# plus-rkwitt/flooder

Measured on AMD Instinct MI355X. Metric: M points×simplices/s (coverage sweep), higher is better.
Workload: dtype f32; 1 GPU; 1M-point 3D Gaussian, 1k landmarks, points_per_edge 30, max_dimension 3, fp32 coverage sweep (BASELINE.json configs[1]); points=1000000, landmarks=1000, top_simplices=6052, top_simplices_rank0=6052, swept_dimension=3, method=cell, parallelism=single GPU

## Files before the change

### flooder_amd/_native.py

```python

from __future__ import annotations

import ctypes
import os
from ctypes import c_char_p, c_float, c_int, c_int32, c_int64, c_uint32, c_void_p

_PKG_DIR = os.path.dirname(os.path.abspath(__file__))
LIB_PATH = os.environ.get("FLOODER_HIP_LIB") or os.path.join(_PKG_DIR, "libflooder_hip.so")



class _Block(ctypes.Structure):

    ABI = 1

    def __init__(self, **fields):
        super().__init__()
        self.size = ctypes.sizeof(self)
        self.abi = self.ABI
        known = {name for name, _ in self._fields_}
        for key, value in fields.items():
            if key not in known:
                raise TypeError(f"{type(self).__name__} has no field {key!r}")
            if value is not None and not isinstance(value, (int, float)):
# ... 8 lines not shown
        item = item.strip()
        if item:
            kind, name = item.split()
            out.append((name, kinds[kind]))
    return out


class FusedSweep(_Block):

    _fields_ = _fields("""u32 size; u32 abi; p pts_sorted; i64 n_pts; i32 dim; i32 k1; p nodes; p density_grid; p cloud_box;
        p verts; p weights; i32 R; i32 n_faces; i64 n_simplices; p memb; f32 alpha; i32 n_coarse; p coarse_rows; p parents;
        p face_bits; p face_slot; p d2_scratch; p flag_list; p flag_count; p flag_key; p flag_hist; p flag_sorted; p top;
        p top_list; p top_count; p simplex_weight; p plane_scratch; p wit_queue; p wit_item_list; p wit_stats;
        p cell_queue; p defer_list; p defer_c; p defer_ctl; p light_list; p heavy_list; p cell_stats; p finish_ctl;
        p hard_scratch; i32 hard_cap; i32 probed; p finish_stats; p wit_runs; i32 wit_run_len; i32 wit_n_runs;
        i32 planes_ready; i32 reserved; p face_owner; p min_face; p chunk_faces; p tile_faces""")


class SortedSweep(_Block):

    _fields_ = _fields("""u32 size; u32 abi; p pts_sorted; i64 n_pts; i32 dim; i32 k1; p nodes; p verts; p weights; i32 R;
        i32 n_faces; i64 n_simplices; p sample_order; p queue; p memb; p face_bits; p face_slot; p stats; p out_d2;
        i32 shard_rank; i32 shard_world""")


class FpsBatched(_Block):

    _fields_ = _fields("""u32 size; u32 abi; p pts; i64 n_pts; i32 dim; i32 ld; p pts_sorted; p order; i64 start; i32 n_lms;
        i32 reserved; p out_idx; p minsq; p bucket_box; p bucket_keys; p bucket_coord; p work_best; p work_rec; p work_ctr;
        p launches_out""")

# ... 291 lines not shown
```

### flooder_amd/core.py

```python

from __future__ import annotations

import ctypes
import itertools
import math
import os
import weakref
import warnings
from numbers import Integral, Real
from typing import Callable, Dict, List, NamedTuple, Optional, Tuple, Union

import numpy as np
import torch

from . import _native
from .simplex_tree import HAS_GUDHI, SimplexTree, delaunay_cells, delaunay_simplices

__all__ = ["flood_complex", "generate_landmarks", "generate_grid", "generate_uniform_weights",
           "SUPPORTED_DTYPES", "HAS_HIP_KERNELS", "PointIndex", "index_from_host"]

SUPPORTED_DTYPES = (torch.float32, torch.float64)
INF_BITS = 0x7F800000
CAND_ALIGN = 8
SWEEP_CHUNK = 2048
# ... 859 lines not shown
    par = (nn[:, 0] | (nn[:, 1] << 8) | (nn[:, 2] << 16) | (nn[:, 3] << 24)).astype(np.uint32)
    rows = np.full(WIT_MAX_COARSE, -1, dtype=np.int32)
    rows[:coarse.size] = inv[coarse]
    out = (rows, np.ascontiguousarray(par[np.asarray(perm)]), int(coarse.size))
    if len(_WIT_PLAN_CACHE) >= 32:
        _WIT_PLAN_CACHE.clear()
    _WIT_PLAN_CACHE[key] = out
    return out


WIT_RUN_LEN = 8
WIT_RUN_SUM_TOL = 2.0 ** -21


def witness_runs(w_perm: np.ndarray, memb: np.ndarray, parents: np.ndarray,
                 run_len: Optional[int] = None) -> Optional[np.ndarray]:
    run_len = WIT_RUN_LEN if run_len is None else int(run_len)
    w32 = np.ascontiguousarray(w_perm, dtype=np.float32)
    R, k1 = w32.shape
    n = R // run_len
    if k1 > 4 or n == 0 or run_len < 8 or run_len & (run_len - 1) or (w32 < 0).any():
        return None
    w = w32.astype(np.float64)[:n * run_len].reshape(n, run_len, k1)
    c = w.mean(axis=1)
    rows = np.arange(n)
    for it in range(1, 65):
        far = ((w - c[:, None, :]) ** 2).sum(axis=2).argmax(axis=1)
        c += (w[rows, far] - c) / (it + 1)
    c32 = np.maximum(c, 0.0).astype(np.float32)
    c64 = c32.astype(np.float64)
    d = np.sqrt(((w - c64[:, None, :]) ** 2).sum(axis=2))
    rho = d.max(axis=1) * (1.0 + 1e-12)
    rho32 = rho.astype(np.float32)
    rho32 = np.where(rho32.astype(np.float64) < rho, np.nextafter(rho32, np.float32(np.inf)), rho32).astype(np.float32)
    sums = w32.astype(np.float64).sum(axis=1)
    if max(np.abs(sums - 1.0).max(), np.abs(c64.sum(axis=1) - 1.0).max()) > 0.5 * WIT_RUN_SUM_TOL:
        return None
    out = np.zeros((n, 8), dtype=np.uint32)
    out[:, :k1] = c32.view(np.uint32)
    out[:, 4] = np.bitwise_or.reduce(np.asarray(memb).view(np.uint32)[:n * run_len].reshape(n, run_len), axis=1)
    out[:, 5] = np.asarray(parents).view(np.uint32)[:n * run_len].reshape(n, run_len)[rows, d.argmin(axis=1)]
    out[:, 6] = rho32.view(np.uint32)
    return out


def face_lattice(weights: np.ndarray, f_ptr: np.ndarray, f_rows: np.ndarray) -> Optional[Tuple[np.ndarray, np.ndarray]]:
    w = np.asarray(weights)
    R, k1 = w.shape
    F = len(f_ptr) - 1
    if F > 32 or k1 > 31:
        return None
    supp = ((w != 0) * (1 << np.arange(k1))).sum(axis=1).astype(np.int64)
    vset = np.array([np.bitwise_or.reduce(supp[f_rows[f_ptr[f]:f_ptr[f + 1]]]) if f_ptr[f + 1] > f_ptr[f] else 0
                     for f in range(F)], dtype=np.int64)
    if len(set(vset.tolist())) != F or (vset == 0).any():
        return None
    holds = (supp[:, None] & ~vset[None, :]) == 0
# ... 78 lines not shown
        if not self._wit_built:
            self._wit_built = True
            wp = witness_plan(self._weights, self._perm) if self.memb_all is not None else None
            if wp is not None:
                dev = self._weights.device
                self._wit = (torch.as_tensor(wp[0], device=dev), torch.as_tensor(wp[1].view(np.int32), device=dev), wp[2])
        return self._wit


    @property
    def wit_runs(self):
        if not self._wit_runs_built:
            self._wit_runs_built = True
            if self.wit is not None:
                run_len = WIT_RUN_LEN
                tab = witness_runs(self.w_perm.cpu().numpy(), self.memb_all.cpu().numpy(), self.wit[1].cpu().numpy(), run_len)
                if tab is not None:
                    self._wit_runs = (torch.as_tensor(tab.view(np.int32), device=self._weights.device), run_len,
                                      int(tab.shape[0]))
        return self._wit_runs


def _sweep_dimension_f64(index: PointIndex, pts64_sorted: torch.Tensor, verts: torch.Tensor, weights: torch.Tensor,
                         faces: _FaceTable, reduce_hook: Optional[Callable[[torch.Tensor], None]],
                         want_dist: bool = False, timer: Optional[_KernelTimer] = None):
    lib = _native.load()
    dev = index.pts.device
    st = _native.current_stream_ptr(dev)
    S, k1, _ = verts.shape
    R = weights.shape[0]
    verts = verts.to(torch.float64).contiguous()
# ... 488 lines not shown
BVH_SORTED_MIN_SAMPLES = 64 * 1024
EMPTY_CACHE_ABOVE_BYTES = 1 << 30
CELL_ALPHA = 1.35
FUSED_FACES = True
CELL_PROBE = True
SHARED_FACE_SLOTS = True
FINISH_HARD_CAP = 32768
CELL_DENSITY_GRID = True
CELL_SUPER = True
WIT_MIN_SIMPLICES = 1536
WIT_MAX_POINTS_PER_SIMPLEX = 400
CELL_WITNESS = True
WIT_RUNS = True
FACE_OWNER = True
FACE_OWNER_GROUPED = False

CTL_FLAG_COUNT, CTL_DEFER, CTL_HIST = 1, 12, 48


def fused_layout(S: int, n_slots: int, wit: bool, owner: bool) -> Tuple[Dict[str, Tuple[int, int]], int]:
    sizes = [("wit_queue", QUEUE_WORDS)] if wit else []
    sizes += [("cell_queue", _native.CELL_QUEUE_WORDS), ("finish_ctl", _native.FINISH_CTL_WORDS), ("top", 2 * S),
              ("ctl", CTL_HIST + _native.FLAG_HIST_WORDS), ("face_bits", n_slots)]
    if owner:
        sizes += [("face_owner", 2 * n_slots), ("result", n_slots)]
    regions, n_words = {}, 0
    for name, words in sizes:
        if name == "face_owner":
            n_words += n_words & 1
        regions[name] = (n_words, words)
# ... 79 lines not shown
                                                              k1, S, _native.ptr(ws.wgt), _native.ptr(ws.planes),
                                                              _native.ptr(ws.arena), ws.n_words, st),
                              "flooder_simplex_prepare_f32")
            else:
                _native.check(lib.flooder_simplex_weight_f32(_native.ptr(index.nodes), index.n, index.dim, _native.ptr(verts),
                                                             k1, S, _native.ptr(ws.wgt), st), "flooder_simplex_weight_f32")
        wst = stats[16:40] if use_wit and stats is not None and stats.numel() >= 40 else None
        blk = _native.FusedSweep(
            pts_sorted=index.pts, n_pts=index.n, dim=index.dim, k1=k1, nodes=index.nodes, density_grid=index.dens,
            cloud_box=index.box, verts=verts, weights=w_perm, R=R, n_faces=F, n_simplices=S, memb=plan.memb_all,
            alpha=float(CELL_ALPHA), face_slot=slot_t, cell_stats=sub(0, 9), probed=1 if CELL_PROBE else 0,
            finish_stats=sub(9, 16), **ws.block_fields())
        if use_owner:
            blk.min_face = plan.min_face.data_ptr()
            blk.chunk_faces, blk.tile_faces = plan.chunk_faces.data_ptr(), plan.tile_faces.data_ptr()
        if use_wit:
            blk.n_coarse, blk.coarse_rows, blk.parents = plan.wit[2], plan.wit[0].data_ptr(), plan.wit[1].data_ptr()
            blk.wit_stats = _native.ptr(wst) or None
            if WIT_RUNS and plan.wit_runs is not None:
                blk.wit_runs, blk.wit_run_len, blk.wit_n_runs = plan.wit_runs[0].data_ptr(), plan.wit_runs[1], plan.wit_runs[2]
        blk.planes_ready = 1 if CELL_SUPER and SWEEP_PREPARE_FUSED else 0
        with _span(timer, "sweep"):
            if use_wit:
                _native.check(lib.flooder_fused_witness(ctypes.byref(blk), st), "flooder_fused_witness")
                blk.planes_ready = 1
            _native.check(lib.flooder_fused_cell(ctypes.byref(blk), st), "flooder_fused_cell")
        with _span(timer, "fallback"):
            _native.check(lib.flooder_fused_finish(ctypes.byref(blk), st), "flooder_fused_finish")
        if stats is not None:
            c_d = ws.defer_ctl[:_native.DEFER_CTL_WORDS].tolist()
# ... 420 lines not shown
```

### flooder_amd/csrc/flood_cell.hip

```cpp

#include <type_traits>

#include "flood_common.hpp"
#include "flood_bvh.hpp"
#include "flood_planes.hpp"

using namespace flooder;

namespace {

constexpr int SPL_CHUNK = 4;
#ifndef FLOODER_CELL_CAPW
#define FLOODER_CELL_CAPW 480
#endif
#ifndef FLOODER_CELL_MAXLEAF
#define FLOODER_CELL_MAXLEAF 584
#endif
#ifndef FLOODER_CELL_WAVES
#define FLOODER_CELL_WAVES 4
#endif
#ifndef FLOODER_CELL_COMPACT
#define FLOODER_CELL_COMPACT 0
#endif
constexpr int CAPW = FLOODER_CELL_CAPW;
// ... 1499 lines not shown
int launch_simplex_planes(int dim, const float* verts, int k1, int64_t n_simplices, float* tab, hipStream_t st) {
  if (dim == 2)
    hipLaunchKernelGGL((simplex_planes_kernel<2>), dim3((unsigned)((n_simplices + 255) / 256)), dim3(256), 0, st, verts, k1,
                       n_simplices, tab);
  else if (dim == 3)
    hipLaunchKernelGGL((simplex_planes_kernel<3>), dim3((unsigned)((n_simplices + 255) / 256)), dim3(256), 0, st, verts, k1,
                       n_simplices, tab);
  else
    return fail(FLOODER_E_ARG, "simplex planes: only dim 2 and 3");
  return check_launch("simplex_planes");
}
}

namespace {

struct OwnerJob {
  unsigned long long* owner = nullptr;
  const int32_t* slot = nullptr;
  int n_faces = 0;
};
__device__ __forceinline__ void choose_owners(const OwnerJob& oj, const float* __restrict__ weight, int n, int block,
                                              int n_blocks, int tid, int nt) {
  const int64_t total = (int64_t)n * oj.n_faces;
  for (int64_t t = (int64_t)block * nt + tid; t < total; t += (int64_t)n_blocks * nt) {
    const int s = (int)(t / oj.n_faces);
    if (t - (int64_t)s * oj.n_faces == 0) continue;
    atomicMax(&oj.owner[oj.slot[t]], owner_key(s, weight[s]));
  }
}
inline int owner_blocks(const OwnerJob& oj, int n, int nt) {
  if (!oj.owner) return 0;
  const int64_t b = ((int64_t)n * oj.n_faces + 4 * nt - 1) / (4 * nt);
  return (int)(b < 1 ? 1 : (b > 1024 ? 1024 : b));
}

__global__ __launch_bounds__(1024) void split_simplices_kernel(const float* __restrict__ weight, int n, float limit,
                                                               float sparse_limit, int32_t* __restrict__ light,
                                                               int32_t* __restrict__ heavy, int32_t* __restrict__ counts,
                                                               OwnerJob oj) {
  if (blockIdx.x > 0) {
    choose_owners(oj, weight, n, (int)blockIdx.x - 1, (int)gridDim.x - 1, (int)threadIdx.x, 1024);
    return;
  }
  __shared__ int s_cl[16], s_ch[16];
  __shared__ int s_sparse, s_act;
  const int lane = threadIdx.x & 63, wv = threadIdx.x >> 6;
  if (threadIdx.x == 0) { s_sparse = 0; s_act = 0; }
  __syncthreads();
  int mine = 0, act = 0;
// ... 230 lines not shown
int flooder::fused_cell(const flooder_fused_sweep_t& a, void* stream) {
  if (a.n_simplices == 0 || a.R == 0) return FLOODER_OK;
  if (!a.memb || !a.face_bits || a.n_faces < 1 || a.n_faces > 32 || (a.top && (!a.top_list || !a.top_count)) ||
      (a.defer_list && (!a.defer_c || !a.defer_ctl)) ||
      (a.simplex_weight && (!a.defer_list || !a.light_list || !a.heavy_list)) || (a.flag_key && (!a.flag_hist || !a.top)) ||
      a.n_simplices > 0x7fffffffLL)
    return fail(FLOODER_E_ARG, "flooder_sweep_cell_faces_f32: bad argument");
  const float* const weight = a.simplex_weight;
  int32_t* const light = weight ? a.light_list : nullptr;
  int32_t* const heavy = weight ? a.heavy_list : nullptr;
  int32_t* const split = weight ? a.defer_ctl + FLOODER_DEFER_CTL_LIGHT : nullptr;
  const int n = (int)a.n_simplices;
  const hipStream_t st = (hipStream_t)stream;
  if (a.face_owner && (!weight || !a.face_slot || !a.min_face || !a.chunk_faces || !a.tile_faces))
    return fail(FLOODER_E_ARG, "flooder_fused_cell: face_owner needs simplex_weight, face_slot, min_face, chunk_faces and tile_faces");
  OwnerJob oj;
  if (a.face_owner) { oj.owner = reinterpret_cast<unsigned long long*>(a.face_owner); oj.slot = a.face_slot; oj.n_faces = a.n_faces; }
  if (weight) {
    const bool long_queue = a.n_simplices * (int64_t)((a.R + 255) / 256) >= (int64_t)g_cell_super_min_chunks;
    if (long_queue && (g_cell_split_launches == 2 || a.n_simplices > 7680)) {
      hipLaunchKernelGGL(split_simplices_kernel, dim3(1 + owner_blocks(oj, n, 1024)), dim3(1024), 0, st, weight, n,
                         (float)g_cell_super_weight, (float)g_cell_super_sparse, light, heavy, split, oj);
      if (g_cell_weight_classes)
        hipLaunchKernelGGL(class_order_kernel<SPLIT_THREADS>, dim3(1), dim3(SPLIT_THREADS), 0, st, weight, n,
                           (float)g_cell_super_weight, (float)g_cell_super_sparse, 2, 1, light, heavy, split, OwnerJob{});
    } else if (long_queue) {
      hipLaunchKernelGGL(class_order_kernel<SPLIT_THREADS_LONG>, dim3(1 + owner_blocks(oj, n, SPLIT_THREADS_LONG)),
                         dim3(SPLIT_THREADS_LONG), 0, st, weight, n, (float)g_cell_super_weight, (float)g_cell_super_sparse,
                         (g_cell_weight_classes ? 2 : 0) | 1 | 4, 0, light, heavy, split, oj);
    } else {
      hipLaunchKernelGGL(class_order_kernel<SPLIT_THREADS>, dim3(1 + owner_blocks(oj, n, SPLIT_THREADS)), dim3(SPLIT_THREADS), 0,
                         st, weight, n, (float)g_cell_super_weight, (float)g_cell_super_sparse, g_cell_weight_classes ? 2 : 0,
                         0, light, heavy, split, oj);
    }
  }
  DeferList dl{a.defer_list, a.defer_c, a.defer_list ? a.defer_ctl + FLOODER_DEFER_CTL_COUNT : nullptr, light, heavy,
               split, g_cell_super_n0};
  if (a.defer_list) {
    const int64_t n_chunk_slots = a.n_simplices * (int64_t)((a.R + 255) / 256);
    dl.tile_list = a.defer_list + n_chunk_slots;
    dl.tile_c = a.defer_c + n_chunk_slots;
    dl.tile_count = a.defer_ctl + FLOODER_DEFER_CTL_TILE_COUNT;
  }
  FaceAcc acc{a.memb, a.face_bits, a.n_faces, reinterpret_cast<unsigned long long*>(a.top), a.top_list,
              a.top_count, a.face_slot, a.flag_key, a.flag_hist};
  if (a.face_owner) {
    acc.owner = oj.owner; acc.min_face = a.min_face; acc.chunk_faces = a.chunk_faces; acc.tile_faces = a.tile_faces;
  }
  return sweep_cell_entry(a, acc, dl, "flooder_sweep_cell_faces_f32: bad argument", stream);
}

extern "C" {

int flooder_sweep_cell_f32(const float* pts_sorted, int64_t n_pts, int dim, const float* nodes,
                           const float* verts, const float* weights, int k1, int R, int64_t n_simplices,
                           float alpha, int32_t* queue, uint32_t* out_d2, int32_t* flag_list, int32_t* flag_count,
                           float* plane_scratch, const int32_t* density_grid, const float* cloud_box, uint64_t* stats,
                           void* stream) {
  flooder_fused_sweep_t a{};
  a.pts_sorted = pts_sorted; a.n_pts = n_pts; a.dim = dim; a.nodes = nodes; a.verts = verts; a.weights = weights;
  a.k1 = k1; a.R = R; a.n_simplices = n_simplices; a.alpha = alpha; a.cell_queue = queue; a.d2_scratch = out_d2;
  a.flag_list = flag_list; a.flag_count = flag_count; a.plane_scratch = plane_scratch; a.density_grid = density_grid;
// ... 58 lines not shown
```

### flooder_amd/csrc/flood_common.hpp

```cpp
#pragma once
#include <hip/hip_runtime.h>
#include <stdint.h>
#include <stdio.h>
#include <string.h>

#include <type_traits>

#include "../../include/flooder_hip.h"

namespace flooder {

constexpr uint32_t INF_BITS = 0x7f800000u;

#define FLOODER_OPTION(name, def, lo, hi, desc) extern int g_##name;
#define FLOODER_OPTION_LIST(name, def, desc, ...) extern int g_##name;
#include "flood_options.def"
#undef FLOODER_OPTION
#undef FLOODER_OPTION_LIST
int launch_simplex_planes(int dim, const float* verts, int k1, int64_t n_simplices, float* tab, hipStream_t st);
char* err_buf();
int fail(int code, const char* msg);
int failf(int code, const char* fmt, ...) __attribute__((format(printf, 2, 3), visibility("hidden")));
int check_launch(const char* what);

// ... 189 lines not shown
      mine = (uint32_t)k == ~(uint32_t)s;
    }
    return (uint32_t)__ballot(mine) | 1u;
  }
  __device__ __forceinline__ int64_t slot_of(int64_t s, int f) const {
    return slot ? (int64_t)slot[s * (int64_t)n_faces + f] : s * (int64_t)n_faces + f;
  }
};

__device__ __forceinline__ unsigned long long owner_key(int s, float w) {
  const uint32_t wb = __float_as_uint(w) < 0x7f800000u ? __float_as_uint(w) : 0x7f800000u;
  const uint32_t hi = w < 0.f ? 0xffffffffu : 0x7fffffffu - wb;
  return ((unsigned long long)hi << 32) | (unsigned long long)(~(uint32_t)s);
}

template <template <int> class F, typename... Args>
int dispatch_dim(int dim, Args&&... args) {
  switch (dim) {
    case 1: return F<1>::run(args...);
    case 2: return F<2>::run(args...);
    case 3: return F<3>::run(args...);
    case 4: return F<4>::run(args...);
    case 5: return F<5>::run(args...);
    case 6: return F<6>::run(args...);
    case 7: return F<7>::run(args...);
    case 8: return F<8>::run(args...);
    default: return fail(FLOODER_E_ARG, "dim must be in 1..8");
  }
}

// ... 108 lines not shown
```

### flooder_amd/csrc/flood_wit.hip

```cpp

#include "flood_common.hpp"
#include "flood_bvh.hpp"

using namespace flooder;

namespace {

#ifndef FLOODER_WIT_BLOCKS
#define FLOODER_WIT_BLOCKS 4
#endif
constexpr int WBLOCKS = FLOODER_WIT_BLOCKS;
constexpr int WTHREADS = 256;
constexpr int WWAVES = WTHREADS / 64;
constexpr int WCAP = 960;
constexpr int WLEAF = 1024;
constexpr int WFRONT = 192;
constexpr int WCOARSE = FLOODER_WIT_MAX_COARSE;
constexpr int WFOCUS = 16;
constexpr int WROUNDS = 8;
constexpr int WUR = 256;
constexpr int WQ = 768;
constexpr int WROWS = FLOODER_WIT_MAX_ROWS;
constexpr int UNR = 4;
constexpr int UNRF = 1;
#ifndef FLOODER_WIT_FDEPTH
#define FLOODER_WIT_FDEPTH 1
#endif
constexpr int FDEPTH = FLOODER_WIT_FDEPTH;
constexpr int NBIN = 64;
constexpr int SGRP = 32;
constexpr int PLANE_ROW = 24;
static_assert(WCOARSE == WTHREADS, "one coarse sample per thread");
static_assert(WUR == WTHREADS && WUR >= WCOARSE, "one open sample per thread in the exact pass");

template <int DP>
__device__ __forceinline__ void load_row_at(const float* __restrict__ base, uint32_t byte_off, float (&out)[DP]) {
  load_row<DP>(reinterpret_cast<const float*>(reinterpret_cast<const char*>(base) + (size_t)byte_off), out);
}

__device__ __forceinline__ int lane_rank(unsigned long long m) {
  return __builtin_amdgcn_mbcnt_hi((uint32_t)(m >> 32), __builtin_amdgcn_mbcnt_lo((uint32_t)m, 0));
}

// ... 163 lines not shown
  __shared__ float s_wit[3 * WCOARSE];
  __shared__ int s_hist[NBIN];
  __shared__ uint32_t s_mf[32];
  __shared__ uint32_t s_unres[WROWS / 32];
  __shared__ uint32_t s_tkey[WROWS / 64];
  __shared__ int s_ftile[WROWS / 64];
  __shared__ int s_gn[MAXL + 2];
  __shared__ int s_ctr[4];
  __shared__ uint16_t s_ur_row[WUR];
  __shared__ uint32_t s_ur_best[WUR];
  __shared__ int16_t s_ur_slot[WUR];
  __shared__ float s_ur_p[WUR * 3];
  __shared__ uint16_t s_focus[WFOCUS];
  __shared__ uint32_t s_fx[8];
  __shared__ float s_rg[Region<DIM>::WORDS];
  __shared__ long long s_item;
  __shared__ int s_off;
  __shared__ float s_run[2];
  __shared__ int s_nrun;
  __shared__ int s_cur[NBIN];
  __shared__ float s_gc[(WCAP + SGRP - 1) / SGRP + 2];
  uint16_t* s_runs = reinterpret_cast<uint16_t*>(s_leaf);
  static_assert(WLEAF * sizeof(int) >= (WROWS / 8) * sizeof(uint16_t), "the run list fits the leaf list (runs of 8 rows or more)");
  uint32_t* s_qub = s_qbuf;
  uint16_t* s_qrow = reinterpret_cast<uint16_t*>(s_qbuf + WQ);
  float4* s_xb = reinterpret_cast<float4*>(s_qbuf);
  constexpr int XB = 256;
  static_assert(XB * sizeof(float4) <= sizeof(uint32_t) * (WQ + WQ / 2) && XB == WTHREADS, "a batch fits the queue's storage");
  const int tid = threadIdx.x;
  const int lane = tid & 63;
  const int wv = tid >> 6;
  const int top = lv.n_levels - 1;
  const int tiles64 = (R + 63) >> 6;
  if (__builtin_amdgcn_readfirstlane(item_count[0]) == 0) return;
  __shared__ unsigned long long s_stat[24];
  enum { ST_HANDLED = 0, ST_HEAVY = 1, ST_OVER = 2, ST_DENSE = 3, ST_STAGED = 4, ST_CCERT = 5, ST_LIVE = 6, ST_ROUNDS = 7,
         ST_UNRES = 8, ST_FLAGGED = 9, ST_PAIRS = 10, ST_BINS = 11, ST_RUNS = 21, ST_EXACT = 22, ST_EXACT_OVER = 23 };
  if (threadIdx.x < 24) s_stat[threadIdx.x] = 0ull;
  auto count = [&](int what, unsigned long long n) {
    if (stats) atomicAdd(&s_stat[what], n);
  };

#ifdef FLOODER_WIT_TIMERS
  unsigned long long t_ph[10] = {0, 0, 0, 0, 0, 0, 0, 0, 0, 0};
  unsigned long long t_prev = __builtin_amdgcn_s_memtime();
#define WPHASE(i) do { const unsigned long long t_ = __builtin_amdgcn_s_memtime(); t_ph[i] += t_ - t_prev; t_prev = t_; } while (0)
#else
#define WPHASE(i) do {} while (0)
#endif
  int q_shard = (int)(blockIdx.x % QSHARDS), q_tried = 0;
  for (;;) {
    WPHASE(8);
// ... 65 lines not shown
#pragma unroll
        for (int k = 0; k < DIM; ++k) {
          float row = 0.f;
#pragma unroll
          for (int l = 0; l < DIM; ++l) {
            float g = 0.f;
#pragma unroll
            for (int j = 0; j < 4; ++j) g = __builtin_fmaf(wn[j][k] * inv, wn[j][l] * inv, g);
            row += __builtin_fabsf(g);
          }
          sig2 = __builtin_fmaxf(sig2, row);
        }
        s_run[0] = sc >= 1e-30f ? __builtin_sqrtf(sig2) * sc * 1.00001f : (sc == 0.f ? 0.f : __builtin_inff());
        s_run[1] = 2.f * rg.epsb;
      }
    }
    if (!(c_max > 0.f) || !(c_max < 3.0e38f)) WIT_ABANDON(ST_OVER)
    __syncthreads();

    float qlo[DIM], qhi[DIM];
    constexpr int GB = 4;
    auto test_children = [&](int lvl, const int (&grp)[GB], int ng, int* out_list, int* out_n, int cap) {
      const int lvl_count = (int)lv.count[lvl], lvl_off = (int)lv.off[lvl];
      bool hit[GB];
      float lo[GB][DP], hi[GB][DP];
#pragma unroll
      for (int u = 0; u < GB; ++u) {
        const int idx = grp[u] * FAN + lane;
        hit[u] = u < ng && idx < lvl_count;
        const uint32_t nb_ = (uint32_t)(lvl_off + (hit[u] ? idx : 0)) * (uint32_t)(2 * DP * sizeof(float));
// ... 451 lines not shown
    WPHASE(4);
    WIT_REC(5, s_ctr[3]);
    if (!(flags & 4)) {
      if (s_ctr[3] > max_open) WIT_ABANDON(ST_DENSE)
      const bool ok = focus_rounds(s_ctr[3], true);
      if (!ok) WIT_ABANDON(ST_DENSE)
      __syncthreads();
    }
    if (tid == 0) s_ctr[3] = 0;
    __syncthreads();
    WPHASE(4);

    struct FineRows {
      float4 w4[UNRF];
      uint32_t par[UNRF], mb[UNRF];
      int rr[UNRF];
      bool valid[UNRF];
    };
    const int run_shift = plan.run_shift;
    int n_run_rows = 0, tail0 = 0;
    if (plan.n_runs > 0) {
      const float sigma = s_run[0], a_abs = s_run[1];
      auto load_run = [&](int i0, uint4& ra, uint4& rb) {
        const int i = i0 + tid < plan.n_runs ? i0 + tid : 0;
        ra = plan.runs[2 * i];
        rb = plan.runs[2 * i + 1];
      };
      uint4 ra_next, rb_next;
      load_run(0, ra_next, rb_next);
      for (int i0 = 0; i0 < plan.n_runs; i0 += WTHREADS) {
        if (i0 + (wv << 6) >= plan.n_runs) break;
        const int i = i0 + tid;
        const bool valid = i < plan.n_runs;
        const uint4 ra = ra_next, rb = rb_next;
        if (i0 + WTHREADS < plan.n_runs) load_run(i0 + WTHREADS, ra_next, rb_next);
        const float cw[4] = {__uint_as_float(ra.x), __uint_as_float(ra.y), __uint_as_float(ra.z), __uint_as_float(ra.w)};
        float g[DIM];
#pragma unroll
        for (int k = 0; k < DIM; ++k) g[k] = 0.f;
#pragma unroll
        for (int j = 0; j < 4; ++j) {
          if (j < k1) {
#pragma unroll
            for (int k = 0; k < DIM; ++k) g[k] = __builtin_fmaf(cw[j], vs[j * DIM + k], g[k]);
          }
        }
        float dg2 = __builtin_inff();
#pragma unroll
        for (int j = 0; j < 4; ++j) {
          const int c = (int)((rb.y >> (8 * j)) & 0xffu);
          float t0 = g[0] - s_wit[3 * c + 0];
          float d2 = t0 * t0;
          t0 = g[1] - s_wit[3 * c + 1];
          d2 = __builtin_fmaf(t0, t0, d2);
          if constexpr (DIM == 3) {
            t0 = g[2] - s_wit[3 * c + 2];
            d2 = __builtin_fmaf(t0, t0, d2);
          }
          dg2 = __builtin_fminf(dg2, d2);
        }
        const float t = __builtin_sqrtf(dg2) + __builtin_fmaf(__uint_as_float(rb.z), sigma, a_abs);
        float bnd = (t * t) * 1.000004f;
        if (bnd < 1e-30f) bnd = __builtin_inff();
        const uint32_t thr = threshold(valid ? rb.x : 0u);
        const bool keep = valid && !(__float_as_uint(bnd) <= thr);
        const unsigned long long m = __ballot(keep);
        if (m != 0ull) {
          int base = 0;
          if (lane == 0) base = atomicAdd(&s_nrun, __popcll(m));
          base = wave_uniform(base);
          if (keep) s_runs[base + lane_rank(m)] = (uint16_t)i;
        }
        if (stats) { const unsigned long long md = __ballot(valid && !keep); if (lane == 0) count(ST_RUNS, (unsigned long long)__popcll(md)); }
      }
      __syncthreads();
      n_run_rows = s_nrun << run_shift;
      tail0 = plan.n_runs << run_shift;
    }
    const int n_fine = n_run_rows + (R - tail0);
    auto load_rows = [&](int g0, FineRows& fr) {
#pragma unroll
      for (int u = 0; u < UNRF; ++u) {
        const int idx = g0 + u * WTHREADS + tid;
        fr.valid[u] = idx < n_fine;
        const int r = !fr.valid[u] ? R - 1
                      : idx < n_run_rows ? ((int)s_runs[idx >> run_shift] << run_shift) + (idx & ((1 << run_shift) - 1))
                                         : tail0 + (idx - n_run_rows);
        fr.rr[u] = r;
        if (k1 == 4) fr.w4[u] = *reinterpret_cast<const float4*>(weights + (int64_t)fr.rr[u] * 4);
        fr.par[u] = plan.parents[fr.rr[u]];
        fr.mb[u] = fr.valid[u] ? acc.memb[fr.rr[u]] : 0u;
      }
    };
    FineRows ring[FDEPTH];
#pragma unroll
    for (int a = 0; a < FDEPTH; ++a)
      if (a * WTHREADS * UNRF < n_fine) load_rows(a * WTHREADS * UNRF, ring[a]);
    for (int g0 = 0; g0 < n_fine; g0 += WTHREADS * UNRF) {
      const FineRows cur = ring[0];
#pragma unroll
      for (int a = 0; a + 1 < FDEPTH; ++a) ring[a] = ring[a + 1];
      if (g0 + FDEPTH * WTHREADS * UNRF < n_fine) load_rows(g0 + FDEPTH * WTHREADS * UNRF, ring[FDEPTH - 1]);
#pragma unroll
      for (int u = 0; u < UNRF; ++u) {
        if (g0 + u * WTHREADS >= n_fine) break;
        float p[DIM];
// ... 11 lines not shown
        }
        float ub = __builtin_inff();
#pragma unroll
        for (int j = 0; j < 4; ++j) {
          const int c = (int)((cur.par[u] >> (8 * j)) & 0xffu);
          float t0 = p[0] - s_wit[3 * c + 0];
          float d2 = t0 * t0;
          t0 = p[1] - s_wit[3 * c + 1];
          d2 = __builtin_fmaf(t0, t0, d2);
          if constexpr (DIM == 3) {
            t0 = p[2] - s_wit[3 * c + 2];
            d2 = __builtin_fmaf(t0, t0, d2);
          }
          ub = __builtin_fminf(ub, d2);
        }
        const uint32_t thr = threshold(cur.mb[u]);
        const bool live = cur.valid[u] && __float_as_uint(ub) > thr;
        const unsigned long long m = __ballot(live);
        if (m != 0ull) {
          int base = 0;
          if (lane == 0) base = atomicAdd(&s_ctr[1], __popcll(m));
          base = wave_uniform(base);
          if (live) {
            const int pos = base + lane_rank(m);
            if (pos < WQ) {
              s_qub[pos] = __float_as_uint(ub);
              s_qrow[pos] = (uint16_t)cur.rr[u];
            } else {
              to_finish(cur.rr[u], ub);
            }
          }
          if (lane == 0) count(ST_LIVE, (unsigned long long)__popcll(m));
// ... 145 lines not shown
    }
    WIT_REC(10, 1); WIT_REC(11, __builtin_amdgcn_s_memrealtime() - t_item0); WIT_REC(7, s_ctr[2]);
    if (tid == 0) { out.weight[s] = -1.f; if ((s & 7) == 0) atomicAdd(&queue[8], 1); }
    if (tid == 0) count(ST_HANDLED, 1);
    WPHASE(7);
  }
  __syncthreads();
  if (stats) {
#ifdef FLOODER_WIT_TIMERS
    if (tid == 0)
      for (int i = 0; i < 10; ++i) atomicAdd(&stats[12 + i], t_ph[i]);
#endif
#ifdef FLOODER_WIT_TIMERS
    const bool flush = tid < 12 || tid >= 22;
#else
    const bool flush = tid < 12 || tid >= ST_RUNS;
#endif
    if (tid < 24 && flush && s_stat[tid] != 0ull) atomicAdd(&stats[tid], s_stat[tid]);
  }
}

constexpr int WCLASSES = 4;
constexpr int WLIST_LDS = 8192;
__global__ __launch_bounds__(1024) void wit_list_kernel(const float* __restrict__ weight, int n, float limit,
                                                        int32_t* __restrict__ list, int32_t* __restrict__ count,
                                                        const int32_t* __restrict__ kind, int surface_pct) {
  __shared__ int s_cnt[WCLASSES][16];
  __shared__ float s_w[WLIST_LDS];
  const int lane = threadIdx.x & 63, wv = threadIdx.x >> 6;
  if (kind != nullptr) {
    const int inner = kind[2], all = kind[3];
    if (all > 0 && (long long)inner * 100 < (long long)all * surface_pct) {
      if (threadIdx.x == 0) count[0] = 0;
      return;
    }
  }
  auto cls = [&](float w) -> int {
    if (!(w >= 0.f) || !(w <= limit)) return -1;
    return w > 0.5f * limit ? 0 : (w > 0.25f * limit ? 1 : (w > 0.125f * limit ? 2 : 3));
  };
  const bool staged = n <= WLIST_LDS;
  if (staged) {
#pragma unroll
    for (int u = 0; u < WLIST_LDS / 1024; ++u) {
      const int i = u * 1024 + (int)threadIdx.x;
      if (i < n) s_w[i] = weight[i];
    }
    __syncthreads();
  }
  const int per = ((n + 1023) / 1024) | 1;
  const int i0 = (int)threadIdx.x * per < n ? (int)threadIdx.x * per : n;
  const int i1 = i0 + per < n ? i0 + per : n;
  int cnt[WCLASSES];
// ... 105 lines not shown
    for (int k = 0; k <= NBIN; ++k) l[k] = Region<DIM>::limit(dl, (float)k / bin_scale);
  }
}

template <int DIM>
struct WitOp {
  static int run(const flooder_fused_sweep_t& a, const Levels& lv, WitPlan plan, WitOut out, FaceAcc acc,
                 const int32_t* kind, hipStream_t st) {
    if constexpr (DIM == 2 || DIM == 3) {
      const int64_t ns = a.n_simplices;
      int32_t* item_count = a.wit_queue + FLOODER_WIT_QUEUE_ITEM_COUNT;
      if (!a.planes_ready) {
        const int rc = launch_simplex_planes(DIM, a.verts, a.k1, ns, a.plane_scratch, st);
        if (rc != FLOODER_OK) return rc;
      }
      hipLaunchKernelGGL(wit_list_kernel, dim3(1), dim3(1024), 0, st, out.weight, (int)ns, (float)g_wit_weight, a.wit_item_list,
                         item_count, g_wit_surface_pct > 0 ? kind : nullptr, g_wit_surface_pct);
      const int grid = (int)(ns < g_wit_grid ? ns : g_wit_grid);
      const int R = a.R;
      hipLaunchKernelGGL((wit_sweep_kernel<DIM>), dim3(grid), dim3(WTHREADS), 0, st, a.pts_sorted, a.nodes, lv, a.verts, a.plane_scratch, a.weights, a.k1,
                         R, ns, (float)g_wit_weight, 0.01f * (float)g_wit_cmax_pct, 0.01f * (float)g_wit_cmax_ext_pct, g_wit_min_bins, g_wit_flags, g_wit_max_open, (int)((int64_t)R * g_wit_max_live_pct / 100), (int)((int64_t)R * g_wit_max_in_pct / 100), g_wit_adaptive, g_wit_max_leaves < WLEAF ? g_wit_max_leaves : WLEAF, g_wit_max_eval, g_wit_sorted_stage, a.wit_item_list, item_count, plan, a.wit_queue, out, acc,
                         reinterpret_cast<unsigned long long*>(a.wit_stats));
      return check_launch("wit_sweep");
    } else {
      return fail(FLOODER_E_ARG, "flooder_sweep_witness_f32: only dim 2 and 3");
    }
  }
};

}

int flooder::fused_witness(const flooder_fused_sweep_t& a, void* stream) {
  if (a.n_simplices == 0 || a.R == 0) return FLOODER_OK;
  if (!a.pts_sorted || !a.nodes || !a.verts || !a.weights || !a.coarse_rows || !a.parents || !a.wit_queue || !a.d2_scratch ||
      !a.memb || !a.face_bits || !a.flag_list || !a.flag_count || !a.simplex_weight || !a.wit_item_list || !a.plane_scratch ||
      a.n_pts < 1 || a.k1 < 1 || a.k1 > FLOODER_MAX_VERTS || a.R < 1 || a.R > WROWS || a.n_coarse < 1 || a.n_coarse > WCOARSE ||
      a.n_faces < 1 || a.n_faces > 32 || (a.top && (!a.top_list || !a.top_count)) || (a.flag_key && !a.flag_hist) ||
      a.n_simplices > 0x7fffffffLL)
    return fail(FLOODER_E_ARG, "flooder_sweep_witness_f32: bad argument");
  if (a.dim != 2 && a.dim != 3) return fail(FLOODER_E_ARG, "flooder_sweep_witness_f32: only dim 2 and 3");
  if (a.n_simplices * (int64_t)((a.R + 63) / 64) > 0x7fffffffLL)
    return fail(FLOODER_E_ARG, "flooder_sweep_witness_f32: too many (simplex, tile) pairs");
  const Levels lv = make_levels(a.n_pts);
  if ((a.n_pts + FLOODER_BVH_LEAF) * (int64_t)(padded_dim(a.dim) * sizeof(float)) >= (1LL << 32) ||
      total_nodes(lv) * (int64_t)(2 * padded_dim(a.dim) * sizeof(float)) >= (1LL << 32))
    return fail(FLOODER_E_ARG, "flooder_sweep_witness_f32: cloud too large");
  const bool have_runs = a.wit_runs && a.wit_n_runs > 0;
  int run_shift = 0;
  if (have_runs) {
    const int run_len = a.wit_run_len;
    if (run_len < 8 || run_len > a.R || (run_len & (run_len - 1)) != 0 || (int64_t)a.wit_n_runs * run_len > a.R || a.k1 > 4)
      return fail(FLOODER_E_ARG, "flooder_fused_witness: bad run table");
    while ((1 << run_shift) < run_len) ++run_shift;
  }
  const bool use_runs = have_runs && g_wit_runs != 0;
  return dispatch_dim<WitOp>(
      a.dim, a, lv,
      WitPlan{a.coarse_rows, a.parents, a.n_coarse, use_runs ? reinterpret_cast<const uint4*>(a.wit_runs) : nullptr,
              run_shift, use_runs ? a.wit_n_runs : 0},
      WitOut{a.d2_scratch, a.flag_list, a.flag_count, a.simplex_weight},
      FaceAcc{a.memb, a.face_bits, a.n_faces, reinterpret_cast<unsigned long long*>(a.top), a.top_list, a.top_count,
              a.face_slot, a.flag_key, a.flag_hist},
      a.density_grid ? a.density_grid + (flooder_density_grid_words(a.dim) - KIND_WORDS) : nullptr, (hipStream_t)stream);
}

extern "C" {

int flooder_wit_max_rows(void) { return WROWS; }
int flooder_wit_max_coarse(void) { return WCOARSE; }

int flooder_sweep_witness_f32(const float* pts_sorted, int64_t n_pts, int dim, const float* nodes, const float* verts,
                              const float* weights, int k1, int R, int64_t n_simplices, const int32_t* coarse_rows,
                              int n_coarse, const uint32_t* parents, int32_t* queue, uint32_t* d2_scratch,
                              const uint32_t* memb, int n_faces, uint32_t* face_bits, const int32_t* face_slot,
                              int32_t* flag_list, int32_t* flag_count, uint32_t* flag_key, int32_t* flag_hist,
                              uint64_t* top, int32_t* top_list, int32_t* top_count, float* simplex_weight,
                              int32_t* item_list, float* plane_scratch, uint64_t* stats, void* stream) {
// ... 39 lines not shown
```

### include/flooder_hip.h

```cpp
#ifndef FLOODER_HIP_H
#define FLOODER_HIP_H

#include <stdint.h>

#ifdef __cplusplus
extern "C" {
#endif

#define FLOODER_ABI_VERSION 1

#define FLOODER_OK 0
#define FLOODER_E_ARG (-1)
#define FLOODER_E_LAUNCH (-2)
#define FLOODER_E_DEVICE (-3)

#define FLOODER_MAX_DIM 8
#define FLOODER_MAX_VERTS 9
#define FLOODER_CAND_ALIGN 8
#define FLOODER_SWEEP_CHUNK 2048
#define FLOODER_TILE_SAMPLES 512
#define FLOODER_BVH_LEAF 16
#define FLOODER_BVH_FANOUT 64
#define FLOODER_BVH_MAX_LEVELS 6
#define FLOODER_QUEUE_SHARDS 16
// ... 253 lines not shown
  int32_t* defer_list;
  float* defer_c;
  int32_t* defer_ctl;
  int32_t* light_list;
  int32_t* heavy_list;
  uint64_t* cell_stats;
  int32_t* finish_ctl;
  uint64_t* hard_scratch;
  int32_t hard_cap;
  int32_t probed;
  uint64_t* finish_stats;
  const uint32_t* wit_runs;
  int32_t wit_run_len;
  int32_t wit_n_runs;
  int32_t planes_ready;
  int32_t reserved;
  uint64_t* face_owner;
  const uint8_t* min_face;
  const uint32_t* chunk_faces;
  const uint32_t* tile_faces;
} flooder_fused_sweep_t;

int flooder_fused_witness(const flooder_fused_sweep_t* p, void* stream);
int flooder_fused_cell(const flooder_fused_sweep_t* p, void* stream);
int flooder_fused_finish(const flooder_fused_sweep_t* p, void* stream);

typedef struct flooder_sorted_sweep_s {
  uint32_t size, abi;
  const float* pts_sorted;
  int64_t n_pts;
  int32_t dim;
// ... 260 lines not shown
```

Before: 6.649 million M points×simplices/s.

## Extend face-owner dedup to witness sweep, skipping rows of foreign faces

Moves owner election into the witness list kernel, using extra blocks beside the list-building block. Owner keys now favour witness candidates. The witness sweep reads a per-simplex owner mask and skips run entries and fine rows whose minimal face belongs to another simplex. Run tables gain a per-run min-face bitmask so whole runs can be skipped. This cuts redundant distance work on shared faces, at the cost of extra per-row loads, more owner atomics and a larger list-kernel grid.

After: 6.683 million M points×simplices/s, median of 6. No clear change (+0.5%).

```diff
diff --git a/flooder_amd/_native.py b/flooder_amd/_native.py
--- a/flooder_amd/_native.py
+++ b/flooder_amd/_native.py
@@ -46,7 +46,7 @@
         p top_list; p top_count; p simplex_weight; p plane_scratch; p wit_queue; p wit_item_list; p wit_stats;
         p cell_queue; p defer_list; p defer_c; p defer_ctl; p light_list; p heavy_list; p cell_stats; p finish_ctl;
         p hard_scratch; i32 hard_cap; i32 probed; p finish_stats; p wit_runs; i32 wit_run_len; i32 wit_n_runs;
-        i32 planes_ready; i32 reserved; p face_owner; p min_face; p chunk_faces; p tile_faces""")
+        i32 planes_ready; i32 owner_mode; p face_owner; p min_face; p chunk_faces; p tile_faces""")
 
 
 class SortedSweep(_Block):
diff --git a/flooder_amd/core.py b/flooder_amd/core.py
--- a/flooder_amd/core.py
+++ b/flooder_amd/core.py
@@ -897,7 +897,7 @@
 
 
 def witness_runs(w_perm: np.ndarray, memb: np.ndarray, parents: np.ndarray,
-                 run_len: Optional[int] = None) -> Optional[np.ndarray]:
+                 run_len: Optional[int] = None, min_face: Optional[np.ndarray] = None) -> Optional[np.ndarray]:
     run_len = WIT_RUN_LEN if run_len is None else int(run_len)
     w32 = np.ascontiguousarray(w_perm, dtype=np.float32)
     R, k1 = w32.shape
@@ -924,6 +924,9 @@
     out[:, 4] = np.bitwise_or.reduce(np.asarray(memb).view(np.uint32)[:n * run_len].reshape(n, run_len), axis=1)
     out[:, 5] = np.asarray(parents).view(np.uint32)[:n * run_len].reshape(n, run_len)[rows, d.argmin(axis=1)]
     out[:, 6] = rho32.view(np.uint32)
+    if min_face is not None:
+        bits = np.left_shift(np.uint32(1), np.asarray(min_face)[:n * run_len].astype(np.uint32))
+        out[:, 7] = np.bitwise_or.reduce(bits.reshape(n, run_len), axis=1)
     return out
 
 
@@ -1032,7 +1035,8 @@
             self._wit_runs_built = True
             if self.wit is not None:
                 run_len = WIT_RUN_LEN
-                tab = witness_runs(self.w_perm.cpu().numpy(), self.memb_all.cpu().numpy(), self.wit[1].cpu().numpy(), run_len)
+                tab = witness_runs(self.w_perm.cpu().numpy(), self.memb_all.cpu().numpy(), self.wit[1].cpu().numpy(), run_len,
+                                   self.min_face.cpu().numpy() if self.min_face is not None else None)
                 if tab is not None:
                     self._wit_runs = (torch.as_tensor(tab.view(np.int32), device=self._weights.device), run_len,
                                       int(tab.shape[0]))
@@ -1551,6 +1555,7 @@
 WIT_RUNS = True
 FACE_OWNER = True
 FACE_OWNER_GROUPED = False
+FACE_OWNER_WIT = True
 
 CTL_FLAG_COUNT, CTL_DEFER, CTL_HIST = 1, 12, 48
 
@@ -1660,6 +1665,7 @@
         if use_owner:
             blk.min_face = plan.min_face.data_ptr()
             blk.chunk_faces, blk.tile_faces = plan.chunk_faces.data_ptr(), plan.tile_faces.data_ptr()
+            blk.owner_mode = 1 if use_wit and FACE_OWNER_WIT else 0
         if use_wit:
             blk.n_coarse, blk.coarse_rows, blk.parents = plan.wit[2], plan.wit[0].data_ptr(), plan.wit[1].data_ptr()
             blk.wit_stats = _native.ptr(wst) or None
diff --git a/flooder_amd/csrc/flood_cell.hip b/flooder_amd/csrc/flood_cell.hip
--- a/flooder_amd/csrc/flood_cell.hip
+++ b/flooder_amd/csrc/flood_cell.hip
@@ -1537,25 +1537,6 @@
 
 namespace {
 
-struct OwnerJob {
-  unsigned long long* owner = nullptr;
-  const int32_t* slot = nullptr;
-  int n_faces = 0;
-};
-__device__ __forceinline__ void choose_owners(const OwnerJob& oj, const float* __restrict__ weight, int n, int block,
-                                              int n_blocks, int tid, int nt) {
-  const int64_t total = (int64_t)n * oj.n_faces;
-  for (int64_t t = (int64_t)block * nt + tid; t < total; t += (int64_t)n_blocks * nt) {
-    const int s = (int)(t / oj.n_faces);
-    if (t - (int64_t)s * oj.n_faces == 0) continue;
-    atomicMax(&oj.owner[oj.slot[t]], owner_key(s, weight[s]));
-  }
-}
-inline int owner_blocks(const OwnerJob& oj, int n, int nt) {
-  if (!oj.owner) return 0;
-  const int64_t b = ((int64_t)n * oj.n_faces + 4 * nt - 1) / (4 * nt);
-  return (int)(b < 1 ? 1 : (b > 1024 ? 1024 : b));
-}
 
 __global__ __launch_bounds__(1024) void split_simplices_kernel(const float* __restrict__ weight, int n, float limit,
                                                                float sparse_limit, int32_t* __restrict__ light,
@@ -1816,8 +1797,10 @@
   const hipStream_t st = (hipStream_t)stream;
   if (a.face_owner && (!weight || !a.face_slot || !a.min_face || !a.chunk_faces || !a.tile_faces))
     return fail(FLOODER_E_ARG, "flooder_fused_cell: face_owner needs simplex_weight, face_slot, min_face, chunk_faces and tile_faces");
+  if (a.owner_mode != 0 && (a.owner_mode != 1 || !a.face_owner))
+    return fail(FLOODER_E_ARG, "flooder_fused_cell: owner_mode must be 0, or 1 with face_owner");
   OwnerJob oj;
-  if (a.face_owner) { oj.owner = reinterpret_cast<unsigned long long*>(a.face_owner); oj.slot = a.face_slot; oj.n_faces = a.n_faces; }
+  if (a.face_owner && a.owner_mode == 0) { oj.owner = reinterpret_cast<unsigned long long*>(a.face_owner); oj.slot = a.face_slot; oj.n_faces = a.n_faces; }
   if (weight) {
     const bool long_queue = a.n_simplices * (int64_t)((a.R + 255) / 256) >= (int64_t)g_cell_super_min_chunks;
     if (long_queue && (g_cell_split_launches == 2 || a.n_simplices > 7680)) {
@@ -1847,7 +1830,7 @@
   FaceAcc acc{a.memb, a.face_bits, a.n_faces, reinterpret_cast<unsigned long long*>(a.top), a.top_list,
               a.top_count, a.face_slot, a.flag_key, a.flag_hist};
   if (a.face_owner) {
-    acc.owner = oj.owner; acc.min_face = a.min_face; acc.chunk_faces = a.chunk_faces; acc.tile_faces = a.tile_faces;
+    acc.owner = reinterpret_cast<unsigned long long*>(a.face_owner); acc.min_face = a.min_face; acc.chunk_faces = a.chunk_faces; acc.tile_faces = a.tile_faces;
   }
   return sweep_cell_entry(a, acc, dl, "flooder_sweep_cell_faces_f32: bad argument", stream);
 }
diff --git a/flooder_amd/csrc/flood_common.hpp b/flooder_amd/csrc/flood_common.hpp
--- a/flooder_amd/csrc/flood_common.hpp
+++ b/flooder_amd/csrc/flood_common.hpp
@@ -227,6 +227,41 @@
   return ((unsigned long long)hi << 32) | (unsigned long long)(~(uint32_t)s);
 }
 
+__device__ __forceinline__ bool wit_candidate(float w, float limit) { return w >= 0.f && w <= limit; }
+__device__ __forceinline__ bool wit_stands_back(const int32_t* __restrict__ kind, int surface_pct) {
+  if (kind == nullptr) return false;
+  const int inner = kind[2], all = kind[3];
+  return all > 0 && (long long)inner * 100 < (long long)all * surface_pct;
+}
+__device__ __forceinline__ unsigned long long owner_key_wit(int s, float w, bool candidate) {
+  const uint32_t wb = __float_as_uint(w) < 0x7f800000u ? __float_as_uint(w) : 0x7f800000u;
+  const uint32_t hi = (candidate ? 0x80000000u : 0u) | (0x7fffffffu - wb);
+  return ((unsigned long long)hi << 32) | (unsigned long long)(~(uint32_t)s);
+}
+
+struct OwnerJob {
+  unsigned long long* owner = nullptr;
+  const int32_t* slot = nullptr;
+  int n_faces = 0;
+};
+__device__ __forceinline__ void choose_owners(const OwnerJob& oj, const float* __restrict__ weight, int n, int block,
+                                              int n_blocks, int tid, int nt, float wit_limit = -1.f,
+                                              bool stands_back = false) {
+  const int64_t total = (int64_t)n * oj.n_faces;
+  for (int64_t t = (int64_t)block * nt + tid; t < total; t += (int64_t)n_blocks * nt) {
+    const int s = (int)(t / oj.n_faces);
+    if (t - (int64_t)s * oj.n_faces == 0) continue;
+    const float w = weight[s];
+    atomicMax(&oj.owner[oj.slot[t]],
+              wit_limit < 0.f ? owner_key(s, w) : owner_key_wit(s, w, !stands_back && wit_candidate(w, wit_limit)));
+  }
+}
+inline int owner_blocks(const OwnerJob& oj, int n, int nt) {
+  if (!oj.owner) return 0;
+  const int64_t b = ((int64_t)n * oj.n_faces + 4 * nt - 1) / (4 * nt);
+  return (int)(b < 1 ? 1 : (b > 1024 ? 1024 : b));
+}
+
 template <template <int> class F, typename... Args>
 int dispatch_dim(int dim, Args&&... args) {
   switch (dim) {
diff --git a/flooder_amd/csrc/flood_wit.hip b/flooder_amd/csrc/flood_wit.hip
--- a/flooder_amd/csrc/flood_wit.hip
+++ b/flooder_amd/csrc/flood_wit.hip
@@ -27,6 +27,9 @@
 #define FLOODER_WIT_FDEPTH 1
 #endif
 constexpr int FDEPTH = FLOODER_WIT_FDEPTH;
+#ifndef FLOODER_WIT_OWNER
+#define FLOODER_WIT_OWNER 1
+#endif
 constexpr int NBIN = 64;
 constexpr int SGRP = 32;
 constexpr int PLANE_ROW = 24;
@@ -220,6 +223,7 @@
   __shared__ uint16_t s_focus[WFOCUS];
   __shared__ uint32_t s_fx[8];
   __shared__ float s_rg[Region<DIM>::WORDS];
+  __shared__ uint32_t s_own;
   __shared__ long long s_item;
   __shared__ int s_off;
   __shared__ float s_run[2];
@@ -241,7 +245,8 @@
   if (__builtin_amdgcn_readfirstlane(item_count[0]) == 0) return;
   __shared__ unsigned long long s_stat[24];
   enum { ST_HANDLED = 0, ST_HEAVY = 1, ST_OVER = 2, ST_DENSE = 3, ST_STAGED = 4, ST_CCERT = 5, ST_LIVE = 6, ST_ROUNDS = 7,
-         ST_UNRES = 8, ST_FLAGGED = 9, ST_PAIRS = 10, ST_BINS = 11, ST_RUNS = 21, ST_EXACT = 22, ST_EXACT_OVER = 23 };
+         ST_UNRES = 8, ST_FLAGGED = 9, ST_PAIRS = 10, ST_BINS = 11, ST_RUNS = 21, ST_EXACT = 22, ST_EXACT_OVER = 23,
+         ST_ROWS4B = 12, ST_SKIP_ROWS = 13, ST_SKIP_LIVE = 14, ST_SKIP_RUNS = 15 };
   if (threadIdx.x < 24) s_stat[threadIdx.x] = 0ull;
   auto count = [&](int what, unsigned long long n) {
     if (stats) atomicAdd(&s_stat[what], n);
@@ -337,6 +342,13 @@
         s_run[0] = sc >= 1e-30f ? __builtin_sqrtf(sig2) * sc * 1.00001f : (sc == 0.f ? 0.f : __builtin_inff());
         s_run[1] = 2.f * rg.epsb;
       }
+    }
+    if (wv == 0) {
+      uint32_t own = 0xffffffffu;
+#if FLOODER_WIT_OWNER
+      if (acc.owner) own = acc.own_mask(s, lane);
+#endif
+      if (lane == 0) s_own = own;
     }
     if (!(c_max > 0.f) || !(c_max < 3.0e38f)) WIT_ABANDON(ST_OVER)
     __syncthreads();
@@ -818,9 +830,17 @@
     struct FineRows {
       float4 w4[UNRF];
       uint32_t par[UNRF], mb[UNRF];
+#if FLOODER_WIT_OWNER
+      uint32_t mf[UNRF];
+#endif
       int rr[UNRF];
       bool valid[UNRF];
     };
+#ifdef FLOODER_WIT_OWNER_COUNTS
+    const bool skip_foreign = !(flags & 16);
+#else
+    constexpr bool skip_foreign = true;
+#endif
     const int run_shift = plan.run_shift;
     int n_run_rows = 0, tail0 = 0;
     if (plan.n_runs > 0) {
@@ -835,7 +855,7 @@
       for (int i0 = 0; i0 < plan.n_runs; i0 += WTHREADS) {
         if (i0 + (wv << 6) >= plan.n_runs) break;
         const int i = i0 + tid;
-        const bool valid = i < plan.n_runs;
+        const bool in_table = i < plan.n_runs;
         const uint4 ra = ra_next, rb = rb_next;
         if (i0 + WTHREADS < plan.n_runs) load_run(i0 + WTHREADS, ra_next, rb_next);
         const float cw[4] = {__uint_as_float(ra.x), __uint_as_float(ra.y), __uint_as_float(ra.z), __uint_as_float(ra.w)};
@@ -866,6 +886,15 @@
         const float t = __builtin_sqrtf(dg2) + __builtin_fmaf(__uint_as_float(rb.z), sigma, a_abs);
         float bnd = (t * t) * 1.000004f;
         if (bnd < 1e-30f) bnd = __builtin_inff();
+#if FLOODER_WIT_OWNER
+        const bool foreign = in_table && rb.w != 0u && (rb.w & s_own) == 0u;
+#else
+        const bool foreign = false;
+#endif
+#ifdef FLOODER_WIT_OWNER_COUNTS
+        if (stats) { const unsigned long long mf_ = __ballot(foreign); if (lane == 0 && mf_ != 0ull) count(ST_SKIP_RUNS, (unsigned long long)__popcll(mf_)); }
+#endif
+        const bool valid = in_table && !(skip_foreign && foreign);
         const uint32_t thr = threshold(valid ? rb.x : 0u);
         const bool keep = valid && !(__float_as_uint(bnd) <= thr);
         const unsigned long long m = __ballot(keep);
@@ -894,6 +923,9 @@
         if (k1 == 4) fr.w4[u] = *reinterpret_cast<const float4*>(weights + (int64_t)fr.rr[u] * 4);
         fr.par[u] = plan.parents[fr.rr[u]];
         fr.mb[u] = fr.valid[u] ? acc.memb[fr.rr[u]] : 0u;
+#if FLOODER_WIT_OWNER
+        fr.mf[u] = acc.owner ? (uint32_t)acc.min_face[fr.rr[u]] : 0u;
+#endif
       }
     };
     FineRows ring[FDEPTH];
@@ -935,8 +967,25 @@
           }
           ub = __builtin_fminf(ub, d2);
         }
-        const uint32_t thr = threshold(cur.mb[u]);
-        const bool live = cur.valid[u] && __float_as_uint(ub) > thr;
+#if FLOODER_WIT_OWNER
+        const bool foreign = cur.valid[u] && !((s_own >> cur.mf[u]) & 1u);
+#else
+        const bool foreign = false;
+#endif
+        const bool swept = cur.valid[u] && !(skip_foreign && foreign);
+        const uint32_t thr = threshold(swept ? cur.mb[u] : 0u);
+        const bool live = swept && __float_as_uint(ub) > thr;
+        if (stats) {
+          const unsigned long long mf_ = __ballot(foreign);
+          if (lane == 0 && mf_ != 0ull) count(ST_SKIP_ROWS, (unsigned long long)__popcll(mf_));
+#ifdef FLOODER_WIT_OWNER_COUNTS
+          const unsigned long long mv_ = __ballot(cur.valid[u]), ml_ = __ballot(foreign && live);
+          if (lane == 0) {
+            count(ST_ROWS4B, (unsigned long long)__popcll(mv_));
+            if (ml_ != 0ull) count(ST_SKIP_LIVE, (unsigned long long)__popcll(ml_));
+          }
+#endif
+        }
         const unsigned long long m = __ballot(live);
         if (m != 0ull) {
           int base = 0;
@@ -1112,7 +1161,7 @@
 #ifdef FLOODER_WIT_TIMERS
     const bool flush = tid < 12 || tid >= 22;
 #else
-    const bool flush = tid < 12 || tid >= ST_RUNS;
+    const bool flush = tid <= ST_SKIP_RUNS || tid >= ST_RUNS;
 #endif
     if (tid < 24 && flush && s_stat[tid] != 0ull) atomicAdd(&stats[tid], s_stat[tid]);
   }
@@ -1122,19 +1171,21 @@
 constexpr int WLIST_LDS = 8192;
 __global__ __launch_bounds__(1024) void wit_list_kernel(const float* __restrict__ weight, int n, float limit,
                                                         int32_t* __restrict__ list, int32_t* __restrict__ count,
-                                                        const int32_t* __restrict__ kind, int surface_pct) {
+                                                        const int32_t* __restrict__ kind, int surface_pct, OwnerJob oj) {
+  if (blockIdx.x > 0) {
+    choose_owners(oj, weight, n, (int)blockIdx.x - 1, (int)gridDim.x - 1, (int)threadIdx.x, 1024, limit,
+                  wit_stands_back(kind, surface_pct));
+    return;
+  }
   __shared__ int s_cnt[WCLASSES][16];
   __shared__ float s_w[WLIST_LDS];
   const int lane = threadIdx.x & 63, wv = threadIdx.x >> 6;
-  if (kind != nullptr) {
-    const int inner = kind[2], all = kind[3];
-    if (all > 0 && (long long)inner * 100 < (long long)all * surface_pct) {
-      if (threadIdx.x == 0) count[0] = 0;
-      return;
-    }
+  if (wit_stands_back(kind, surface_pct)) {
+    if (threadIdx.x == 0) count[0] = 0;
+    return;
   }
   auto cls = [&](float w) -> int {
-    if (!(w >= 0.f) || !(w <= limit)) return -1;
+    if (!wit_candidate(w, limit)) return -1;
     return w > 0.5f * limit ? 0 : (w > 0.25f * limit ? 1 : (w > 0.125f * limit ? 2 : 3));
   };
   const bool staged = n <= WLIST_LDS;
@@ -1270,8 +1321,11 @@
         const int rc = launch_simplex_planes(DIM, a.verts, a.k1, ns, a.plane_scratch, st);
         if (rc != FLOODER_OK) return rc;
       }
-      hipLaunchKernelGGL(wit_list_kernel, dim3(1), dim3(1024), 0, st, out.weight, (int)ns, (float)g_wit_weight, a.wit_item_list,
-                         item_count, g_wit_surface_pct > 0 ? kind : nullptr, g_wit_surface_pct);
+      OwnerJob oj;
+      if (a.owner_mode == 1) { oj.owner = reinterpret_cast<unsigned long long*>(a.face_owner); oj.slot = a.face_slot; oj.n_faces = a.n_faces; }
+      hipLaunchKernelGGL(wit_list_kernel, dim3(1 + owner_blocks(oj, (int)ns, 1024)), dim3(1024), 0, st, out.weight, (int)ns,
+                         (float)g_wit_weight, a.wit_item_list, item_count, g_wit_surface_pct > 0 ? kind : nullptr,
+                         g_wit_surface_pct, oj);
       const int grid = (int)(ns < g_wit_grid ? ns : g_wit_grid);
       const int R = a.R;
       hipLaunchKernelGGL((wit_sweep_kernel<DIM>), dim3(grid), dim3(WTHREADS), 0, st, a.pts_sorted, a.nodes, lv, a.verts, a.plane_scratch, a.weights, a.k1,
@@ -1301,6 +1355,8 @@
   if ((a.n_pts + FLOODER_BVH_LEAF) * (int64_t)(padded_dim(a.dim) * sizeof(float)) >= (1LL << 32) ||
       total_nodes(lv) * (int64_t)(2 * padded_dim(a.dim) * sizeof(float)) >= (1LL << 32))
     return fail(FLOODER_E_ARG, "flooder_sweep_witness_f32: cloud too large");
+  if (a.owner_mode != 0 && (a.owner_mode != 1 || !a.face_owner || !a.face_slot || !a.min_face))
+    return fail(FLOODER_E_ARG, "flooder_fused_witness: owner_mode must be 0, or 1 with face_owner, face_slot and min_face");
   const bool have_runs = a.wit_runs && a.wit_n_runs > 0;
   int run_shift = 0;
   if (have_runs) {
@@ -1310,13 +1366,14 @@
     while ((1 << run_shift) < run_len) ++run_shift;
   }
   const bool use_runs = have_runs && g_wit_runs != 0;
+  FaceAcc acc{a.memb, a.face_bits, a.n_faces, reinterpret_cast<unsigned long long*>(a.top), a.top_list, a.top_count,
+              a.face_slot, a.flag_key, a.flag_hist};
+  if (a.owner_mode == 1) { acc.owner = reinterpret_cast<const unsigned long long*>(a.face_owner); acc.min_face = a.min_face; }
   return dispatch_dim<WitOp>(
       a.dim, a, lv,
       WitPlan{a.coarse_rows, a.parents, a.n_coarse, use_runs ? reinterpret_cast<const uint4*>(a.wit_runs) : nullptr,
               run_shift, use_runs ? a.wit_n_runs : 0},
-      WitOut{a.d2_scratch, a.flag_list, a.flag_count, a.simplex_weight},
-      FaceAcc{a.memb, a.face_bits, a.n_faces, reinterpret_cast<unsigned long long*>(a.top), a.top_list, a.top_count,
-              a.face_slot, a.flag_key, a.flag_hist},
+      WitOut{a.d2_scratch, a.flag_list, a.flag_count, a.simplex_weight}, acc,
       a.density_grid ? a.density_grid + (flooder_density_grid_words(a.dim) - KIND_WORDS) : nullptr, (hipStream_t)stream);
 }
 
diff --git a/include/flooder_hip.h b/include/flooder_hip.h
--- a/include/flooder_hip.h
+++ b/include/flooder_hip.h
@@ -291,7 +291,7 @@
   int32_t wit_run_len;
   int32_t wit_n_runs;
   int32_t planes_ready;
-  int32_t reserved;
+  int32_t owner_mode;
   uint64_t* face_owner;
   const uint8_t* min_face;
   const uint32_t* chunk_faces;
```
